# eugenelet/CRFP

Hardware: AMD Instinct MI355X
Metric: sr_frames_per_sec (higher is better)
Workload: dtype f32; 1 GPU; BASELINE configs[1]: single MI355X, 7-frame 180x320 -> 1440x2560 x8 SR, batch=1, fp32, sigma_T=10; mode=clip, frames_per_clip=7, fv_size=96, clips_per_call=1, calls_in_flight_per_gpu=1, clips_in_flight_per_gpu=1, batching=one clip per call, storage=f32, parallelism=clip-sharded x1

## Files before the change

### crfp_amd/csrc/conv_narrow.hip

```cpp
#include "crfp_common.h"
#include <cstdlib>
#include <cstring>

namespace CRFP_NS {

typedef float f32x4 __attribute__((ext_vector_type(4)));

__device__ __forceinline__ float n_act(float v, int act) {
    switch (act) {
        case CRFP_ACT_RELU: return fmaxf(v, 0.0f);
        case CRFP_ACT_LRELU01: return v > 0.0f ? v : 0.1f * v;
        case CRFP_ACT_TANH: return tanhf(v);
        case CRFP_ACT_SIGMOID: return 1.0f / (1.0f + expf(-v));
        default: return v;
    }
}

constexpr int kNarrowOcc1 = kActBf16 ? 5 : 4;
constexpr int kNarrowOcc2 = 3;
constexpr int kNarrowOcc3 = 2;
constexpr int NTW = 64, NTH = 16, NLW = NTW + 2, NLH = NTH + 2;
constexpr int NST = (NLH * NLW + 255) / 256;

#ifdef CRFP_ACT_BF16
__device__ __forceinline__ cu32x2 raw_flow(const char* p) { return *reinterpret_cast<const cu32x2*>(p); }
__device__ __forceinline__ cu32x2 flow_words(cu32x2 r) {
    typedef __bf16 b2_t __attribute__((ext_vector_type(2)));
    const cf32x2 fl = __builtin_bit_cast(cf32x2, r);
    const b2_t hi = __builtin_convertvector(fl, b2_t);
    const cf32x2 back = __builtin_convertvector(hi, cf32x2);
    const b2_t lo = __builtin_convertvector(cf32x2{fl.x - back.x, fl.y - back.y}, b2_t);
    return cu32x2{__builtin_bit_cast(unsigned, hi), __builtin_bit_cast(unsigned, lo)};
}
__device__ __forceinline__ f32x4 raw_to_quad(cu32x2 r, bool flow) {
    const cf32x2 fl = __builtin_bit_cast(cf32x2, r);
    return flow ? f32x4{fl.x, fl.y, 0.0f, 0.0f} : quad_from_bits(r);
}
#else
__device__ __forceinline__ f32x4 raw_flow(const char* p) {
    const float2 f = *reinterpret_cast<const float2*>(p);
    return f32x4{f.x, f.y, 0.0f, 0.0f};
}
__device__ __forceinline__ f32x4 raw_to_quad(f32x4 r, bool) { return r; }
#endif

__device__ __forceinline__ void narrow_src_index(int dst, float scale, int in_size, int& i0, int& i1, float& l0, float& l1) {
    float src = scale * ((float)dst + 0.5f) - 0.5f;
    if (src < 0.0f) src = 0.0f;
    i0 = min((int)floorf(src), in_size - 1);
    i1 = min(i0 + 1, in_size - 1);
    l1 = fminf(fmaxf(src - (float)i0, 0.0f), 1.0f);
    l0 = 1.0f - l1;
}

__device__ __forceinline__ void narrow_store_state(act_t* d2, long long ppix, cf32x4 v, float& vmax) {
#ifdef CRFP_ACT_BF16
    const cf32x4 u = cf32x4{v.x > 0.0f ? v.x : 0.1f * v.x, v.y > 0.0f ? v.y : 0.1f * v.y, v.z > 0.0f ? v.z : 0.1f * v.z, v.w > 0.0f ? v.w : 0.1f * v.w};
    vmax = fmaxf(fmaxf(vmax, fmaxf(fabsf(u.x), fabsf(u.y))), fmaxf(fabsf(u.z), fabsf(u.w)));
    v = quad_from_bits(quad_to_bits(v));
    stq(d2 + ppix * 4, cf32x4{v.x > 0.0f ? v.x : 0.1f * v.x, v.y > 0.0f ? v.y : 0.1f * v.y, v.z > 0.0f ? v.z : 0.1f * v.z, v.w > 0.0f ? v.w : 0.1f * v.w});
    return;
#endif
    const cf32x4 o = cf32x4{v.x > 0.0f ? v.x : 0.1f * v.x, v.y > 0.0f ? v.y : 0.1f * v.y, v.z > 0.0f ? v.z : 0.1f * v.z, v.w > 0.0f ? v.w : 0.1f * v.w};
    stq(d2 + ppix * 4, o);
    vmax = fmaxf(fmaxf(vmax, fmaxf(fabsf(o.x), fabsf(o.y))), fmaxf(fabsf(o.z), fabsf(o.w)));
}

template <int KQ, int EPI, bool GATE = false, bool ST2 = false>
__global__ __launch_bounds__(256, KQ == 1 ? kNarrowOcc1 : (KQ == 2 ? kNarrowOcc2 : kNarrowOcc3)) void conv3x3_narrow_kernel(const NarrowArgs a) {
#ifdef CRFP_ACT_BF16
    __shared__ cu32x2 tile[KQ][NLH][NLW];
#else
    __shared__ float4 tile[KQ][NLH][NLW];
    __shared__ float4 wl[9 * KQ * 4];
#endif
    const int tid = threadIdx.x, tx = tid & 63, ty = tid >> 6;
#ifndef CRFP_ACT_BF16
    if (tid < 9 * KQ * 4) {
        const float4 wv = reinterpret_cast<const float4*>(a.wpk)[tid];
        float* wf = reinterpret_cast<float*>(wl) + (tid >> 2) * 16 + (tid & 3);
        wf[0] = wv.x; wf[4] = wv.y; wf[8] = wv.z; wf[12] = wv.w;
    }
#endif
    const int n = blockIdx.z;
    const int H = a.H, W = a.W;
    const int tiles_x = (W + NTW - 1) / NTW, ntiles = tiles_x * ((H + NTH - 1) / NTH);

    const char* qbase[KQ];
    int qpitch[KQ];
    bool qflow[KQ];
#pragma unroll
    for (int k = 0; k < KQ; ++k) {
        int kql = k, s = 0;
        while (s < a.nsrc - 1 && kql >= a.src[s].nq) { kql -= a.src[s].nq; ++s; }
        const ConvSrc src = a.src[s];
        qflow[k] = src.kind == SRC_FLOW2;
        qpitch[k] = W + src.pad;
        qbase[k] = qflow[k] ? reinterpret_cast<const char*>(src.p + (long long)n * src.bstride)
                            : reinterpret_cast<const char*>(as_act(src.p) + (long long)n * src.bstride + (long long)kql * (H + src.pad) * qpitch[k] * 4);
    }
#ifdef CRFP_ACT_BF16
    typedef __bf16 nb16x8 __attribute__((ext_vector_type(8)));
    typedef __bf16 nb16x2 __attribute__((ext_vector_type(2)));
    typedef unsigned nu32x4 __attribute__((ext_vector_type(4)));
    nb16x8 aw[KQ][5];
    {
        const int lane = tid & 63, c = lane & 3;
        const bool diag = (lane >> 4) == ((lane & 15) >> 2);
#pragma unroll
        for (int k = 0; k < KQ; ++k)
#pragma unroll
            for (int st = 0; st < 5; ++st) {
                nu32x4 wds;
#pragma unroll
                for (int hf = 0; hf < 2; ++hf) {
                    const int tap = 2 * st + hf;
                    float v[4] = {0.0f, 0.0f, 0.0f, 0.0f};
                    if (tap < 9) {
#pragma unroll
                        for (int comp = 0; comp < 4; ++comp) {
                            const int cc = qflow[k] ? (comp & 1) : comp;
                            const float wv = a.wpk[((tap * KQ + k) * 4 + cc) * 4 + c];
                            v[comp] = diag ? wv : 0.0f;
                        }
                    }
                    wds[2 * hf] = __builtin_bit_cast(unsigned, __builtin_convertvector(cf32x2{v[0], v[1]}, nb16x2));
                    wds[2 * hf + 1] = __builtin_bit_cast(unsigned, __builtin_convertvector(cf32x2{v[2], v[3]}, nb16x2));
                }
                aw[k][st] = __builtin_bit_cast(nb16x8, wds);
            }
    }
#endif
    const float4 bias = *reinterpret_cast<const float4*>(a.bpk);
    const int cout = a.cout, act = a.act;
    const float slope = act == CRFP_ACT_RELU ? 0.0f : (act == CRFP_ACT_LRELU01 ? 0.1f : 1.0f);
    const bool slow_act = act == CRFP_ACT_TANH || act == CRFP_ACT_SIGMOID;
    const float post = a.post_scale;
    float* const dst = a.dst + (long long)n * a.dst_bstride;
    act_t* const dsta = as_act(a.dst) + (long long)n * a.dst_bstride;
    const int dpitch = W + a.dst_pad;
    const act_t* const resid = a.resid ? as_act(a.resid) + (long long)n * a.resid_bstride : nullptr;
    act_t* const dst2 = ST2 ? as_act(a.dst2) + (long long)n * a.dst2_bstride : nullptr;
    const uint8_t* const mask = EPI == NE_BLEND ? a.mask + (long long)n * a.mask_bstride : nullptr;
    const act_t* const basep = EPI == NE_LAST && a.base ? as_act(a.base) + (long long)n * a.base_bstride : nullptr;
    const float* const baselr = EPI == NE_LAST && !a.base ? a.base_lr + (long long)n * a.base_bstride : nullptr;
    unsigned* const ovfw = ovf_word(a.ovf, a.ovf_div, a.ovf_add, n);
    const bool poison = EPI == NE_LAST && ovfw && *ovfw != 0;
    float vmax = 0.0f;
    const float* const flowp = EPI == NE_OFFMASK3 ? a.flow + (long long)n * a.flow_bstride : nullptr;
    const bool y_only = a.y_only != 0;

#ifdef CRFP_ACT_BF16
    typedef cu32x2 rawq_t;
#else
    typedef f32x4 rawq_t;
#endif
#ifdef CRFP_LAB
    const int NPROBE = a.rsv;
#else
    constexpr int NPROBE = 0;
#endif
    rawq_t r[KQ][NST];
    bool okr[NST];
#define CRFP_NARROW_LOAD(T)                                                                               \
    {                                                                                                     \
        const int ty_ = (T) / tiles_x, x0_ = ((T) - ty_ * tiles_x) * NTW, y0_ = ty_ * NTH;                \
        int cgy[NST], cgx[NST];                                                                           \
        _Pragma("unroll") for (int t = 0; t < NST; ++t) {                                                 \
            const int idx = min(tid + 256 * t, NLH * NLW - 1);                                            \
            const int rr = idx / NLW, c = idx - rr * NLW;                                                 \
            const int gy = y0_ + rr - 1, gx = x0_ + c - 1;                                                \
            okr[t] = tid + 256 * t < NLH * NLW && gy >= 0 && gy < H && gx >= 0 && gx < W;                 \
            cgy[t] = min(max(gy, 0), H - 1);                                                              \
            cgx[t] = min(max(gx, 0), W - 1);                                                              \
        }                                                                                                 \
        if (!(NPROBE & 4))                                                                                \
        _Pragma("unroll") for (int k = 0; k < KQ; ++k) {                                                  \
            if (qflow[k]) {                                                             \
                _Pragma("unroll") for (int t = 0; t < NST; ++t)                                           \
                    r[k][t] = raw_flow(qbase[k] + ((long long)cgy[t] * W + cgx[t]) * 8);                  \
            } else {                                                                                      \
                _Pragma("unroll") for (int t = 0; t < NST; ++t)                                           \
                    r[k][t] = *reinterpret_cast<const rawq_t*>(qbase[k] + ((long long)cgy[t] * qpitch[k] + cgx[t]) * kQuadBytes); \
            }                                                                                             \
        }                                                                                                 \
    }

    constexpr bool BAND = EPI != NE_LAST;
    const int xq = ntiles >> 3, xr = ntiles & 7, xcd = blockIdx.x & 7;
    const int band0 = BAND ? xcd * xq + min(xcd, xr) : 0;
    const int band1 = BAND ? band0 + xq + (xcd < xr ? 1 : 0) : ntiles;
    const int t_step = BAND ? ((int)gridDim.x - xcd + 7) >> 3 : (int)gridDim.x;
    int t_cur = BAND ? band0 + (blockIdx.x >> 3) : (int)blockIdx.x;
    const uint8_t* const gate = GATE ? a.gate + (long long)n * a.gate_bstride + a.gate_h : nullptr;
    if (GATE)
        while (t_cur < band1 && !gate[4 * t_cur]) t_cur += t_step;
    if (t_cur >= band1) return;
    CRFP_NARROW_LOAD(t_cur)
    for (;;) {
#pragma unroll
        for (int k = 0; k < KQ; ++k)
#pragma unroll
            for (int t = 0; t < NST; ++t) {
                const int idx = tid + 256 * t;
#ifdef CRFP_ACT_BF16
                if (idx < NLH * NLW) (&tile[k][0][0])[idx] = okr[t] ? (qflow[k] ? flow_words(r[k][t]) : r[k][t]) : cu32x2{0u, 0u};
#else
                if (idx < NLH * NLW) reinterpret_cast<f32x4*>(&tile[k][0][0])[idx] = okr[t] ? raw_to_quad(r[k][t], qflow[k]) : f32x4{0.0f, 0.0f, 0.0f, 0.0f};
#endif
            }
        __syncthreads();
        int t_next = t_cur + t_step;
        if (GATE)
            while (t_next < band1 && !gate[4 * t_next]) t_next += t_step;
        if (t_next < band1) CRFP_NARROW_LOAD(t_next)

        f32x4 acc[4];
#pragma unroll
        for (int i = 0; i < 4; ++i) acc[i] = f32x4{bias.x, bias.y, bias.z, bias.w};
#ifdef CRFP_ACT_BF16
#pragma unroll
        for (int k = 0; k < KQ; ++k)
#pragma unroll
            for (int i = 0; i < 4; ++i)
#pragma unroll
                for (int st = 0; st < 5; ++st) {
                    const int t0 = 2 * st, t1 = 2 * st + 1;
                    const cu32x2 q0 = tile[k][4 * ty + i + t0 / 3][tx + t0 % 3];
                    const cu32x2 q1 = t1 < 9 ? tile[k][4 * ty + i + t1 / 3][tx + t1 % 3] : cu32x2{0u, 0u};
                    acc[i] = __builtin_amdgcn_mfma_f32_16x16x32_bf16(aw[k][st], __builtin_bit_cast(nb16x8, nu32x4{q0.x, q0.y, q1.x, q1.y}),
                                                                     acc[i], 0, 0, 0);
                }
#else
#pragma unroll 1
        for (int k = 0; k < ((NPROBE & 1) ? 0 : KQ); ++k) {
#pragma unroll
            for (int ky = 0; ky < 3; ++ky) {
#pragma unroll
                for (int kx = 0; kx < 3; ++kx) {
                    const float4 wv = wl[((ky * 3 + kx) * KQ + k) * 4 + (tx & 3)];
                    f32x4 u[4];
#pragma unroll
                    for (int i = 0; i < 4; ++i) u[i] = reinterpret_cast<const f32x4&>(tile[k][4 * ty + ky + i][tx + kx]);
#pragma unroll
                    for (int i = 0; i < 4; ++i) acc[i] = __builtin_amdgcn_mfma_f32_4x4x1f32(wv.x, u[i].x, acc[i], 0, 0, 0);
#pragma unroll
                    for (int i = 0; i < 4; ++i) acc[i] = __builtin_amdgcn_mfma_f32_4x4x1f32(wv.y, u[i].y, acc[i], 0, 0, 0);
#pragma unroll
                    for (int i = 0; i < 4; ++i) acc[i] = __builtin_amdgcn_mfma_f32_4x4x1f32(wv.z, u[i].z, acc[i], 0, 0, 0);
#pragma unroll
                    for (int i = 0; i < 4; ++i) acc[i] = __builtin_amdgcn_mfma_f32_4x4x1f32(wv.w, u[i].w, acc[i], 0, 0, 0);
                }
            }
        }
#endif

        const int tyi = t_cur / tiles_x, x = (t_cur - tyi * tiles_x) * NTW + tx, y0 = tyi * NTH;
        if (x < W && !(NPROBE & 2)) {
#pragma unroll
            for (int i = 0; i < 4; ++i) {
                const int y = y0 + 4 * ty + i;
                if (y >= H) break;
                const long long pix = (long long)y * W + x;
                const long long dpix = (long long)y * dpitch + x;
                if (EPI == NE_PLAIN) {
                    float v[4];
                    if (slow_act) {
#pragma unroll
                        for (int o = 0; o < 4; ++o) v[o] = n_act(acc[i][o], act) * post;
                    } else {
#pragma unroll
                        for (int o = 0; o < 4; ++o) v[o] = fmaxf(acc[i][o], slope * acc[i][o]) * post;
                    }
#pragma unroll
                    for (int o = 0; o < 4; ++o)
                        if (o >= cout) v[o] = 0.0f;
                    if (resid) {
                        const cf32x4 rv = ldq(resid + pix * 4);
                        v[0] += rv.x; v[1] += rv.y; v[2] += rv.z; v[3] += rv.w;
                    }
                    stq(dsta + dpix * 4, cf32x4{v[0], v[1], v[2], v[3]});
                    if (ST2) narrow_store_state(dst2, (long long)y * (W + 1) + x, cf32x4{v[0], v[1], v[2], v[3]}, vmax);
                } else if (EPI == NE_BLEND) {
#ifdef CRFP_ACT_BF16
                    const cf32x4 centre = quad_from_bits(tile[0][4 * ty + i + 1][tx + 1]);
#else
                    const float4 centre = tile[0][4 * ty + i + 1][tx + 1];
#endif
                    const bool m = mask[pix] != 0;
                    float v[4] = {m ? acc[i][0] : centre.x, m ? acc[i][1] : centre.y, m ? acc[i][2] : centre.z,
                                  m ? acc[i][3] : centre.w};
#pragma unroll
                    for (int o = 0; o < 4; ++o) v[o] = v[o] > 0.0f ? v[o] : 0.1f * v[o];
                    vmax = fmaxf(fmaxf(vmax, fmaxf(fabsf(v[0]), fabsf(v[1]))), fmaxf(fabsf(v[2]), fabsf(v[3])));
                    stq(dsta + dpix * 4, cf32x4{v[0], v[1], v[2], v[3]});
                } else if (EPI == NE_LAST) {
                    cf32x4 b;
                    if (basep) {
                        b = ldq(basep + pix * 4);
                    } else {
                        const int lh = H >> 3, lw = W >> 3;
                        int y0, y1, x0, x1;
                        float ly0, ly1, lx0, lx1;
                        narrow_src_index(y, 0.125f, lh, y0, y1, ly0, ly1);
                        narrow_src_index(x, 0.125f, lw, x0, x1, lx0, lx1);
                        float u[3];
#pragma unroll
                        for (int c = 0; c < 3; ++c) {
                            const float* p = baselr + (long long)c * lh * lw;
                            u[c] = ly0 * (lx0 * p[y0 * lw + x0] + lx1 * p[y0 * lw + x1]) + ly1 * (lx0 * p[y1 * lw + x0] + lx1 * p[y1 * lw + x1]);
                        }
                        b = cf32x4{u[0], u[1], u[2], 0.0f};
                    }
                    const float bad = poison ? __builtin_nanf("") : 0.0f;
                    if (y_only) {
                        dst[pix] = acc[i][0] + (0.299f * b.x + 0.587f * b.y + 0.114f * b.z) + bad;
                    } else {
                        const long long plane = (long long)H * W;
                        dst[pix] = acc[i][0] + b.x + bad;
                        dst[plane + pix] = acc[i][1] + b.y + bad;
                        dst[2 * plane + pix] = acc[i][2] + b.z + bad;
                    }
                } else {
                    const float2 f = *reinterpret_cast<const float2*>(flowp + pix * 2);
                    *reinterpret_cast<float4*>(dst + dpix * 4) =
                        make_float4(tanh10_plus(acc[i][0], 10.0f + f.y), tanh10_plus(acc[i][1], 10.0f + f.x),
                                    fast_sigmoid(acc[i][2]), 0.0f);
                }
            }
        }
        if ((EPI == NE_BLEND || ST2) && ovfw && !(vmax < 65504.0f)) { atomicOr(ovfw, 1u); vmax = 0.0f; }
        if (t_next >= band1) break;
        t_cur = t_next;
        asm volatile("s_waitcnt lgkmcnt(0)\n\ts_barrier" ::: "memory");
    }
#undef CRFP_NARROW_LOAD
}

#ifndef CRFP_ACT_BF16
template <int KQ>
__global__ __launch_bounds__(256, kNarrowOcc1) void conv3x3_narrow_seq_kernel(const NarrowArgs a) {
    __shared__ float4 tile[NLH][NLW];
    __shared__ float4 wl[9 * KQ * 4];
    const int tid = threadIdx.x, tx = tid & 63, ty = tid >> 6;
    if (tid < 9 * KQ * 4) {
        const float4 wv = reinterpret_cast<const float4*>(a.wpk)[tid];
        float* wf = reinterpret_cast<float*>(wl) + (tid >> 2) * 16 + (tid & 3);
        wf[0] = wv.x; wf[4] = wv.y; wf[8] = wv.z; wf[12] = wv.w;
    }
    const int n = blockIdx.z;
    const int H = a.H, W = a.W;
    const int tiles_x = (W + NTW - 1) / NTW, ntiles = tiles_x * ((H + NTH - 1) / NTH);
    const char* qbase[KQ];
    int qpitch[KQ];
    bool qflow[KQ];
#pragma unroll
    for (int k = 0; k < KQ; ++k) {
        int kql = k, s = 0;
        while (s < a.nsrc - 1 && kql >= a.src[s].nq) { kql -= a.src[s].nq; ++s; }
        const ConvSrc src = a.src[s];
        qflow[k] = src.kind == SRC_FLOW2;
        qpitch[k] = W + src.pad;
        qbase[k] = qflow[k] ? reinterpret_cast<const char*>(src.p + (long long)n * src.bstride)
                            : reinterpret_cast<const char*>(src.p + (long long)n * src.bstride + (long long)kql * (H + src.pad) * qpitch[k] * 4);
    }
    const float4 bias = *reinterpret_cast<const float4*>(a.bpk);
    const int cout = a.cout, act = a.act;
    const float slope = act == CRFP_ACT_RELU ? 0.0f : (act == CRFP_ACT_LRELU01 ? 0.1f : 1.0f);
    const float post = a.post_scale;
    float* const dsta = a.dst + (long long)n * a.dst_bstride;
    const int dpitch = W + a.dst_pad;
    const float* const resid = a.resid ? a.resid + (long long)n * a.resid_bstride : nullptr;
    const bool plain_out = cout == 4 && post == 1.0f;

    f32x4 r[NST];
    bool okr[NST];
    bool r_in = false;
    unsigned hoff[NST];
    bool pitch_w = true;
#pragma unroll
    for (int k = 0; k < KQ; ++k) pitch_w = pitch_w && qpitch[k] == W;
#pragma unroll
    for (int t = 0; t < NST; ++t) {
        const int idx = min(tid + 256 * t, NLH * NLW - 1), rr = idx / NLW;
        hoff[t] = (unsigned)(rr * W + (idx - rr * NLW)) * 16u;
    }
#define CRFP_SEQ_LOAD(T, K_)                                                                              \
    {                                                                                                     \
        const int ty_ = (T) / tiles_x, x0_ = ((T) - ty_ * tiles_x) * NTW, y0_ = ty_ * NTH;                \
        const char* qb_ = qbase[0]; int qp_ = qpitch[0]; bool qf_ = qflow[0];                             \
        _Pragma("unroll") for (int kk = 1; kk < KQ; ++kk)                                                 \
            if ((K_) == kk) { qb_ = qbase[kk]; qp_ = qpitch[kk]; qf_ = qflow[kk]; }                       \
        r_in = pitch_w && x0_ >= 1 && y0_ >= 1 && x0_ + NLW - 1 <= W && y0_ + NLH - 1 <= H;               \
        if (r_in) {    \
            const int so_ = ((y0_ - 1) * W + (x0_ - 1)) * 16;                                             \
            if (qf_) {                                                                                    \
                const __amdgpu_buffer_rsrc_t rs_ = __builtin_amdgcn_make_buffer_rsrc(const_cast<char*>(qb_), 0, H * W * 8, 0x00020000); \
                _Pragma("unroll") for (int t = 0; t < NST; ++t) {                                         \
                    const cf32x2 f_ = __builtin_bit_cast(cf32x2, __builtin_amdgcn_raw_buffer_load_b64(rs_, (int)(hoff[t] >> 1), so_ >> 1, 0)); \
                    r[t] = f32x4{f_.x, f_.y, 0.0f, 0.0f};                                                 \
                }                                                                                         \
            } else {                                                                                      \
                const __amdgpu_buffer_rsrc_t rs_ = __builtin_amdgcn_make_buffer_rsrc(const_cast<char*>(qb_), 0, H * W * 16, 0x00020000); \
                _Pragma("unroll") for (int t = 0; t < NST; ++t)                                           \
                    r[t] = __builtin_bit_cast(f32x4, __builtin_amdgcn_raw_buffer_load_b128(rs_, (int)hoff[t], so_, 0)); \
            }                                                                                             \
        } else {                                                                                          \
            _Pragma("unroll") for (int t = 0; t < NST; ++t) {                                             \
                const int idx_ = min(tid + 256 * t, NLH * NLW - 1), hr_ = idx_ / NLW, hc_ = idx_ - hr_ * NLW; \
                const int gy = y0_ + hr_ - 1, gx = x0_ + hc_ - 1;                                         \
                okr[t] = tid + 256 * t < NLH * NLW && gy >= 0 && gy < H && gx >= 0 && gx < W;             \
                const int cgy = min(max(gy, 0), H - 1), cgx = min(max(gx, 0), W - 1);                     \
                if (qf_) r[t] = raw_flow(qb_ + ((long long)cgy * W + cgx) * 8);                           \
                else r[t] = *reinterpret_cast<const f32x4*>(qb_ + ((long long)cgy * qp_ + cgx) * 16);     \
            }                                                                                             \
        }                                                                                                 \
    }
    const int xq = ntiles >> 3, xr = ntiles & 7, xcd = blockIdx.x & 7;
    const int band0 = xcd * xq + min(xcd, xr), band1 = band0 + xq + (xcd < xr ? 1 : 0);
    const int t_step = ((int)gridDim.x - xcd + 7) >> 3;
    int t_cur = band0 + (blockIdx.x >> 3), k_cur = 0;
    if (t_cur >= band1) return;
    CRFP_SEQ_LOAD(t_cur, 0)
    f32x4 acc[4];
    for (;;) {
        if (r_in) {
#pragma unroll
            for (int t = 0; t < NST; ++t)
                if (256 * t + 255 < NLH * NLW || tid + 256 * t < NLH * NLW) reinterpret_cast<f32x4*>(&tile[0][0])[tid + 256 * t] = r[t];
        } else {
#pragma unroll
            for (int t = 0; t < NST; ++t) {
                const int idx = tid + 256 * t;
                if (idx < NLH * NLW) reinterpret_cast<f32x4*>(&tile[0][0])[idx] = okr[t] ? r[t] : f32x4{0.0f, 0.0f, 0.0f, 0.0f};
            }
        }
        __syncthreads();
        const bool last_k = k_cur == KQ - 1;
        const int t_next = last_k ? t_cur + t_step : t_cur, k_next = last_k ? 0 : k_cur + 1;
        if (t_next < band1) CRFP_SEQ_LOAD(t_next, k_next)
        if (k_cur == 0) {
#pragma unroll
            for (int i = 0; i < 4; ++i) acc[i] = f32x4{bias.x, bias.y, bias.z, bias.w};
        }
#pragma unroll
        for (int ky = 0; ky < 3; ++ky) {
#pragma unroll
            for (int kx = 0; kx < 3; ++kx) {
                const float4 wv = wl[((ky * 3 + kx) * KQ + k_cur) * 4 + (tx & 3)];
                f32x4 u[4];
#pragma unroll
                for (int i = 0; i < 4; ++i) u[i] = reinterpret_cast<const f32x4&>(tile[4 * ty + ky + i][tx + kx]);
#pragma unroll
                for (int i = 0; i < 4; ++i) acc[i] = __builtin_amdgcn_mfma_f32_4x4x1f32(wv.x, u[i].x, acc[i], 0, 0, 0);
#pragma unroll
                for (int i = 0; i < 4; ++i) acc[i] = __builtin_amdgcn_mfma_f32_4x4x1f32(wv.y, u[i].y, acc[i], 0, 0, 0);
#pragma unroll
                for (int i = 0; i < 4; ++i) acc[i] = __builtin_amdgcn_mfma_f32_4x4x1f32(wv.z, u[i].z, acc[i], 0, 0, 0);
#pragma unroll
                for (int i = 0; i < 4; ++i) acc[i] = __builtin_amdgcn_mfma_f32_4x4x1f32(wv.w, u[i].w, acc[i], 0, 0, 0);
            }
        }
        if (last_k) {
            const int tyi = t_cur / tiles_x, x0 = (t_cur - tyi * tiles_x) * NTW, x = x0 + tx, y0 = tyi * NTH;
            if (plain_out && x0 + NTW <= W && y0 + NTH <= H) {
                float* const dt = dsta + ((long long)y0 * dpitch + x0) * 4;
                const float* const rt_ = resid ? resid + ((long long)y0 * W + x0) * 4 : nullptr;
#pragma unroll
                for (int i = 0; i < 4; ++i) {
                    cf32x4 v;
#pragma unroll
                    for (int o = 0; o < 4; ++o) v[o] = fmaxf(acc[i][o], slope * acc[i][o]);
                    if (rt_) {
                        const cf32x4 rv = ldq(rt_ + (unsigned)((4 * ty + i) * W + tx) * 4u);
                        v[0] += rv.x; v[1] += rv.y; v[2] += rv.z; v[3] += rv.w;
                    }
                    stq(dt + (unsigned)((4 * ty + i) * dpitch + tx) * 4u, v);
                }
            } else if (x < W) {
#pragma unroll
                for (int i = 0; i < 4; ++i) {
                    const int y = y0 + 4 * ty + i;
                    if (y >= H) break;
                    float v[4];
#pragma unroll
                    for (int o = 0; o < 4; ++o) v[o] = o < cout ? fmaxf(acc[i][o], slope * acc[i][o]) * post : 0.0f;
                    if (resid) {
                        const cf32x4 rv = ldq(resid + ((long long)y * W + x) * 4);
                        v[0] += rv.x; v[1] += rv.y; v[2] += rv.z; v[3] += rv.w;
                    }
                    stq(dsta + ((long long)y * dpitch + x) * 4, cf32x4{v[0], v[1], v[2], v[3]});
                }
            }
        }
        if (t_next >= band1) break;
        t_cur = t_next; k_cur = k_next;
        asm volatile("s_waitcnt lgkmcnt(0)\n\ts_barrier" ::: "memory");
    }
#undef CRFP_SEQ_LOAD
}
#endif

constexpr int PLW = NTW + 4, PLH = NTH + 4;
constexpr int PMW = NTW + 2, PMH = NTH + 2;
constexpr int PSTA = (PLH * PLW + 255) / 256;
constexpr int PNA = (PMH * PMW + 255) / 256;

template <int KQA, int EPIB>
__global__ __launch_bounds__(256, KQA == 1 ? 3 : 2) void conv3x3_narrow_pair_kernel(const NarrowArgs a, const NarrowArgs b) {
    __shared__ float4 tileA[KQA][PLH][PLW];
    __shared__ float4 tileB[PMH][PMW];
    __shared__ float4 wlA[9 * KQA * 4], wlB[9 * 4];
    const int tid = threadIdx.x, tx = tid & 63, ty = tid >> 6;
    if (tid < 9 * KQA * 4) {
        const float4 wv = reinterpret_cast<const float4*>(a.wpk)[tid];
        float* wf = reinterpret_cast<float*>(wlA) + (tid >> 2) * 16 + (tid & 3);
        wf[0] = wv.x; wf[4] = wv.y; wf[8] = wv.z; wf[12] = wv.w;
    }
    if (tid < 9 * 4) {
        const float4 wv = reinterpret_cast<const float4*>(b.wpk)[tid];
        float* wf = reinterpret_cast<float*>(wlB) + (tid >> 2) * 16 + (tid & 3);
        wf[0] = wv.x; wf[4] = wv.y; wf[8] = wv.z; wf[12] = wv.w;
    }
    const int n = blockIdx.z;
    const int H = a.H, W = a.W;
    const int tiles_x = (W + NTW - 1) / NTW, ntiles = tiles_x * ((H + NTH - 1) / NTH);
    const char* qbase[KQA];
    int qpitch[KQA];
    bool qflow[KQA];
#pragma unroll
    for (int k = 0; k < KQA; ++k) {
        int kql = k, s = 0;
        while (s < a.nsrc - 1 && kql >= a.src[s].nq) { kql -= a.src[s].nq; ++s; }
        const ConvSrc src = a.src[s];
        qflow[k] = src.kind == SRC_FLOW2;
        qpitch[k] = W + src.pad;
        qbase[k] = qflow[k] ? reinterpret_cast<const char*>(src.p + (long long)n * src.bstride)
                            : reinterpret_cast<const char*>(as_act(src.p) + (long long)n * src.bstride + (long long)kql * (H + src.pad) * qpitch[k] * 4);
    }
    const float4 biasA = *reinterpret_cast<const float4*>(a.bpk), biasB = *reinterpret_cast<const float4*>(b.bpk);
    const float slopeA = a.act == CRFP_ACT_RELU ? 0.0f : (a.act == CRFP_ACT_LRELU01 ? 0.1f : 1.0f);
    const float slopeB = b.act == CRFP_ACT_RELU ? 0.0f : (b.act == CRFP_ACT_LRELU01 ? 0.1f : 1.0f);
    const int coutB = b.cout;
    float* const dst = b.dst + (long long)n * b.dst_bstride;
    act_t* const dsta = as_act(b.dst) + (long long)n * b.dst_bstride;
    const int dpitch = W + b.dst_pad;
    const act_t* const resid = b.resid ? as_act(b.resid) + (long long)n * b.resid_bstride : nullptr;
    const float* const flowp = EPIB == NE_OFFMASK3 ? b.flow + (long long)n * b.flow_bstride : nullptr;
    act_t* const dst2 = EPIB == NE_PLAIN && b.dst2 ? as_act(b.dst2) + (long long)n * b.dst2_bstride : nullptr;
    unsigned* const ovfw = dst2 ? ovf_word(b.ovf, b.ovf_div, b.ovf_add, n) : nullptr;
    float vmax = 0.0f;

#ifdef CRFP_ACT_BF16
    typedef cu32x2 rawq_t;
#else
    typedef f32x4 rawq_t;
#endif
    rawq_t r[KQA][PSTA];
    bool okr[PSTA];
#define CRFP_PAIR_LOAD(T)                                                                                 \
    {                                                                                                     \
        const int ty_ = (T) / tiles_x, x0_ = ((T) - ty_ * tiles_x) * NTW, y0_ = ty_ * NTH;                \
        int cgy[PSTA], cgx[PSTA];                                                                         \
        _Pragma("unroll") for (int t = 0; t < PSTA; ++t) {                                                \
            const int idx = min(tid + 256 * t, PLH * PLW - 1);                                            \
            const int rr = idx / PLW, c = idx - rr * PLW;                                                 \
            const int gy = y0_ + rr - 2, gx = x0_ + c - 2;                                                \
            okr[t] = tid + 256 * t < PLH * PLW && gy >= 0 && gy < H && gx >= 0 && gx < W;                 \
            cgy[t] = min(max(gy, 0), H - 1);                                                              \
            cgx[t] = min(max(gx, 0), W - 1);                                                              \
        }                                                                                                 \
        _Pragma("unroll") for (int k = 0; k < KQA; ++k) {                                                 \
            if (qflow[k]) {                                                                               \
                _Pragma("unroll") for (int t = 0; t < PSTA; ++t)                                          \
                    r[k][t] = raw_flow(qbase[k] + ((long long)cgy[t] * W + cgx[t]) * 8);                  \
            } else {                                                                                      \
                _Pragma("unroll") for (int t = 0; t < PSTA; ++t)                                          \
                    r[k][t] = *reinterpret_cast<const rawq_t*>(qbase[k] + ((long long)cgy[t] * qpitch[k] + cgx[t]) * kQuadBytes); \
            }                                                                                             \
        }                                                                                                 \
    }

    const int xq = ntiles >> 3, xr = ntiles & 7, xcd = blockIdx.x & 7;
    const int band0 = xcd * xq + min(xcd, xr), band1 = band0 + xq + (xcd < xr ? 1 : 0);
    const int t_step = ((int)gridDim.x - xcd + 7) >> 3;
    int t_cur = band0 + (blockIdx.x >> 3);
    if (t_cur >= band1) return;
    CRFP_PAIR_LOAD(t_cur)
    for (;;) {
#pragma unroll
        for (int k = 0; k < KQA; ++k)
#pragma unroll
            for (int t = 0; t < PSTA; ++t) {
                const int idx = tid + 256 * t;
                if (idx < PLH * PLW) reinterpret_cast<f32x4*>(&tileA[k][0][0])[idx] = okr[t] ? raw_to_quad(r[k][t], qflow[k]) : f32x4{0.0f, 0.0f, 0.0f, 0.0f};
            }
        __syncthreads();
        const int t_next = t_cur + t_step;
        if (t_next < band1) CRFP_PAIR_LOAD(t_next)
        const int tyi = t_cur / tiles_x, x0 = (t_cur - tyi * tiles_x) * NTW, y0 = tyi * NTH;

        {
            f32x4 acc[PNA];
            int pr[PNA], pc[PNA];
#pragma unroll
            for (int i = 0; i < PNA; ++i) {
                const int idx = min(tid + 256 * i, PMH * PMW - 1);
                pr[i] = idx / PMW; pc[i] = idx - pr[i] * PMW;
                acc[i] = f32x4{biasA.x, biasA.y, biasA.z, biasA.w};
            }
#pragma unroll 1
            for (int k = 0; k < KQA; ++k)
#pragma unroll 1
                for (int ky = 0; ky < 3; ++ky)
#pragma unroll
                    for (int kx = 0; kx < 3; ++kx) {
                        const float4 wv = wlA[((ky * 3 + kx) * KQA + k) * 4 + (tx & 3)];
                        f32x4 u[PNA];
#pragma unroll
                        for (int i = 0; i < PNA; ++i) u[i] = reinterpret_cast<const f32x4&>(tileA[k][pr[i] + ky][pc[i] + kx]);
#pragma unroll
                        for (int i = 0; i < PNA; ++i) acc[i] = __builtin_amdgcn_mfma_f32_4x4x1f32(wv.x, u[i].x, acc[i], 0, 0, 0);
#pragma unroll
                        for (int i = 0; i < PNA; ++i) acc[i] = __builtin_amdgcn_mfma_f32_4x4x1f32(wv.y, u[i].y, acc[i], 0, 0, 0);
#pragma unroll
// ... 705 lines not shown
```

Baseline: 735.7 frames/s.

## Stage low-res base window in LDS for final conv bilinear upsample epilogue

In the last-layer epilogue of the narrow 3x3 conv, the x8 bilinear upsample of the low-res base image used to gather four global values per channel per output pixel. Now a 3-channel 4x10 low-res window is prefetched into a register alongside the tile loads and written to shared memory each tile. The horizontal interpolation is computed once per thread and reused across its four rows, leaving only the vertical blend per row. This cuts scattered global loads and index math in the epilogue, at the cost of a little extra LDS and a register live across the loop. It relies on the four rows a thread owns mapping to the same pair of low-res rows.

After: 740.6 frames/s, median of 6. About the same (+0.7%).

```diff
diff --git a/crfp_amd/csrc/conv_narrow.hip b/crfp_amd/csrc/conv_narrow.hip
--- a/crfp_amd/csrc/conv_narrow.hip
+++ b/crfp_amd/csrc/conv_narrow.hip
@@ -52,6 +52,7 @@
     l1 = fminf(fmaxf(src - (float)i0, 0.0f), 1.0f);
     l0 = 1.0f - l1;
 }
+constexpr int kBaseWinH = 4, kBaseWinW = 10, kBaseWin = 3 * kBaseWinH * kBaseWinW;
 
 __device__ __forceinline__ void narrow_store_state(act_t* d2, long long ppix, cf32x4 v, float& vmax) {
 #ifdef CRFP_ACT_BF16
@@ -74,6 +75,7 @@
     __shared__ float4 tile[KQ][NLH][NLW];
     __shared__ float4 wl[9 * KQ * 4];
 #endif
+    __shared__ float win[EPI == NE_LAST ? kBaseWin : 1];
     const int tid = threadIdx.x, tx = tid & 63, ty = tid >> 6;
 #ifndef CRFP_ACT_BF16
     if (tid < 9 * KQ * 4) {
@@ -184,7 +186,15 @@
                     r[k][t] = *reinterpret_cast<const rawq_t*>(qbase[k] + ((long long)cgy[t] * qpitch[k] + cgx[t]) * kQuadBytes); \
             }                                                                                             \
         }                                                                                                 \
-    }
+        if (EPI == NE_LAST && baselr && !(NPROBE & 4)) {    \
+             \
+            const int ws_ = min(tid, kBaseWin - 1), wc_ = ws_ / (kBaseWinH * kBaseWinW), wr_ = ws_ / kBaseWinW - wc_ * kBaseWinH; \
+            const int wy_ = min(max((y0_ >> 3) - 1 + wr_, 0), lh - 1), wx_ = min(max((x0_ >> 3) - 1 + ws_ % kBaseWinW, 0), lw - 1); \
+            wreg = baselr[(wc_ * lh + wy_) * lw + wx_];                                                   \
+        }                                                                                                 \
+    }
+    const int lh = H >> 3, lw = W >> 3;
+    float wreg = 0.0f;
 
     constexpr bool BAND = EPI != NE_LAST;
     const int xq = ntiles >> 3, xr = ntiles & 7, xcd = blockIdx.x & 7;
@@ -209,6 +219,7 @@
                 if (idx < NLH * NLW) reinterpret_cast<f32x4*>(&tile[k][0][0])[idx] = okr[t] ? raw_to_quad(r[k][t], qflow[k]) : f32x4{0.0f, 0.0f, 0.0f, 0.0f};
 #endif
             }
+        if (EPI == NE_LAST && baselr && tid < kBaseWin) win[tid] = wreg;
         __syncthreads();
         int t_next = t_cur + t_step;
         if (GATE)
@@ -256,7 +267,57 @@
 #endif
 
         const int tyi = t_cur / tiles_x, x = (t_cur - tyi * tiles_x) * NTW + tx, y0 = tyi * NTH;
-        if (x < W && !(NPROBE & 2)) {
+        if (EPI == NE_LAST) {
+            if (x < W && !(NPROBE & 2)) {
+                const float bad = poison ? __builtin_nanf("") : 0.0f;
+                const long long plane = (long long)H * W;
+                auto put = [&](long long pix, const f32x4& v, const cf32x4& b) {
+                    if (y_only) {
+                        dst[pix] = v[0] + (0.299f * b.x + 0.587f * b.y + 0.114f * b.z) + bad;
+                    } else {
+                        dst[pix] = v[0] + b.x + bad;
+                        dst[plane + pix] = v[1] + b.y + bad;
+                        dst[2 * plane + pix] = v[2] + b.z + bad;
+                    }
+                };
+                if (basep) {
+#pragma unroll
+                    for (int i = 0; i < 4; ++i) {
+                        const int y = y0 + 4 * ty + i;
+                        if (y >= H) break;
+                        const long long pix = (long long)y * W + x;
+                        put(pix, acc[i], ldq(basep + pix * 4));
+                    }
+                    __builtin_amdgcn_s_waitcnt(0x0F70);
+                } else {
+                    float bh0[3] = {0.0f, 0.0f, 0.0f}, bh1[3] = {0.0f, 0.0f, 0.0f};
+                    if (!(NPROBE & 8)) {
+                        int by0, by1, bx0, bx1;
+                        float bl0, bl1, lx0, lx1;
+                        narrow_src_index(y0 + 4 * ty, 0.125f, lh, by0, by1, bl0, bl1);
+                        narrow_src_index(x, 0.125f, lw, bx0, bx1, lx0, lx1);
+                        const int wy = (y0 >> 3) - 1, wx = ((x - tx) >> 3) - 1;
+                        const int r0 = (by0 - wy) * kBaseWinW - wx, r1 = (by1 - wy) * kBaseWinW - wx;
+#pragma unroll
+                        for (int c = 0; c < 3; ++c) {
+                            const float* const p = win + c * kBaseWinH * kBaseWinW;
+                            bh0[c] = lx0 * p[r0 + bx0] + lx1 * p[r0 + bx1];
+                            bh1[c] = lx0 * p[r1 + bx0] + lx1 * p[r1 + bx1];
+                        }
+                    }
+#pragma unroll
+                    for (int i = 0; i < 4; ++i) {
+                        const int y = y0 + 4 * ty + i;
+                        if (y >= H) break;
+                        int yi0, yi1;
+                        float ly0, ly1;
+                        narrow_src_index(y, 0.125f, lh, yi0, yi1, ly0, ly1);
+                        put((long long)y * W + x, acc[i],
+                            cf32x4{ly0 * bh0[0] + ly1 * bh1[0], ly0 * bh0[1] + ly1 * bh1[1], ly0 * bh0[2] + ly1 * bh1[2], 0.0f});
+                    }
+                }
+            }
+        } else if (x < W && !(NPROBE & 2)) {
 #pragma unroll
             for (int i = 0; i < 4; ++i) {
                 const int y = y0 + 4 * ty + i;
@@ -294,33 +355,6 @@
                     for (int o = 0; o < 4; ++o) v[o] = v[o] > 0.0f ? v[o] : 0.1f * v[o];
                     vmax = fmaxf(fmaxf(vmax, fmaxf(fabsf(v[0]), fabsf(v[1]))), fmaxf(fabsf(v[2]), fabsf(v[3])));
                     stq(dsta + dpix * 4, cf32x4{v[0], v[1], v[2], v[3]});
-                } else if (EPI == NE_LAST) {
-                    cf32x4 b;
-                    if (basep) {
-                        b = ldq(basep + pix * 4);
-                    } else {
-                        const int lh = H >> 3, lw = W >> 3;
-                        int y0, y1, x0, x1;
-                        float ly0, ly1, lx0, lx1;
-                        narrow_src_index(y, 0.125f, lh, y0, y1, ly0, ly1);
-                        narrow_src_index(x, 0.125f, lw, x0, x1, lx0, lx1);
-                        float u[3];
-#pragma unroll
-                        for (int c = 0; c < 3; ++c) {
-                            const float* p = baselr + (long long)c * lh * lw;
-                            u[c] = ly0 * (lx0 * p[y0 * lw + x0] + lx1 * p[y0 * lw + x1]) + ly1 * (lx0 * p[y1 * lw + x0] + lx1 * p[y1 * lw + x1]);
-                        }
-                        b = cf32x4{u[0], u[1], u[2], 0.0f};
-                    }
-                    const float bad = poison ? __builtin_nanf("") : 0.0f;
-                    if (y_only) {
-                        dst[pix] = acc[i][0] + (0.299f * b.x + 0.587f * b.y + 0.114f * b.z) + bad;
-                    } else {
-                        const long long plane = (long long)H * W;
-                        dst[pix] = acc[i][0] + b.x + bad;
-                        dst[plane + pix] = acc[i][1] + b.y + bad;
-                        dst[2 * plane + pix] = acc[i][2] + b.z + bad;
-                    }
                 } else {
                     const float2 f = *reinterpret_cast<const float2*>(flowp + pix * 2);
                     *reinterpret_cast<float4*>(dst + dpix * 4) =
```
